# jczarnowski/DeepFactors

Measured on NVIDIA H100. Metric: keyframe-pair Jacobian+JtJ evals/sec (640x480, C=32), higher is better.
Workload: dtype f32

## Files before the change

### deepfactors_b200/csrc/dfk_api.cu

```cuda
#include <cuda_runtime.h>
#include <math.h>
#include <stdint.h>
#include <stdio.h>
#include <stdlib.h>
#include <string.h>

#include <algorithm>
#include <memory>
#include <new>
#include <string>
#include <vector>

#include "dfk.h"
#include "dfk_internal.h"

using namespace dfk;

namespace {

template <typename T, bool Pinned>
struct Scratch {
  T* ptr = nullptr;
  size_t cap = 0;

  Scratch() = default;
  Scratch(Scratch&& o) noexcept : ptr(o.ptr), cap(o.cap) { o.ptr = nullptr; o.cap = 0; }
  ~Scratch() { release(); }

  void release()
  {
    if constexpr (Pinned) cudaFreeHost(ptr);
    else cudaFree(ptr);
    ptr = nullptr;
    cap = 0;
  }
  cudaError_t ensure(size_t need)
  {
    if (cap >= need) return cudaSuccess;
    const size_t n = std::max(need, cap * 2);
    release();
    void* p = nullptr;
    const cudaError_t e = Pinned ? cudaMallocHost(&p, n * sizeof(T)) : cudaMalloc(&p, n * sizeof(T));
    if (e != cudaSuccess) return e;
    ptr = static_cast<T*>(p);
    cap = n;
    return e;
  }
};
template <typename T>
using DeviceBuf = Scratch<T, false>;
template <typename T>
using PinnedBuf = Scratch<T, true>;

}

struct DfkContext {
  int device = 0;
  int num_sms = 1;
  int sm_limit = 0;
  cudaStream_t own_stream = nullptr;
  cudaStream_t stream = nullptr;
  std::string err;
  DfkSfmAlignerParams params;
  DfkGramMode gram_mode = DFK_GRAM_AUTO;
  float se3_huber_delta = 0.1f;

  DeviceBuf<float> simple_scratch;
  DeviceBuf<unsigned int> counter;
  DeviceBuf<float> out_dev;
  PinnedBuf<float> out_host;
  DeviceBuf<float> code_dev;
  DeviceBuf<float> track_dev;
  PinnedBuf<float> track_host;
  DeviceBuf<unsigned char> batch_dev;
  PinnedBuf<unsigned char> batch_host;
  DeviceBuf<float> batch_partials;
  DeviceBuf<unsigned int> batch_counters;

  DeviceBuf<float> sparse_dev;
  PinnedBuf<float> sparse_host;
  DeviceBuf<unsigned char> rep_dev;
  std::vector<unsigned char> rep_host;
  DeviceBuf<unsigned char> geo_dev;
  std::vector<unsigned char> geo_host;
  DeviceBuf<SfmItemDev> items_dev;
  DeviceBuf<float> partials_dev;
  struct RayTab {
    float fx, fy, u0, v0;
    uint32_t w, h;
    DeviceBuf<float> dev;
    bool built;
  };
  std::vector<RayTab> ray_cache;
  std::vector<size_t> ray_pending;
  bool ray_flush = false;
  DeviceBuf<float> codes_dev;
  std::vector<float> codes_host;
  DeviceBuf<float> records_dev;
  PinnedBuf<float> records_host;
  std::vector<SfmItemDev> items_host;

  bool profiling = false;
  std::vector<cudaEvent_t> ev_pool;
  size_t ev_used = 0;
  double ev_ms_accum = 0.0;
  uint64_t ev_count_accum = 0;
  uint64_t launches = 0;

  ~DfkContext()
  {
    for (cudaEvent_t e : ev_pool) cudaEventDestroy(e);
    if (own_stream) cudaStreamDestroy(own_stream);
  }
};

struct DfkSfmStream {
  int device = 0, code_size = 0, max_items = 0, depth = 0;
  size_t max_bytes = 0;
  cudaStream_t copy_stream = nullptr;
  struct Slot {
    DeviceBuf<unsigned char> dev;
    DeviceBuf<float> rec_dev;
    PinnedBuf<float> rec_host;
    cudaEvent_t uploaded = nullptr, done = nullptr;
    int n = 0;
    uint64_t ticket = 0;
    bool busy = false;
  };
  std::vector<Slot> slots;
  std::vector<DfkSfmWorkItem> dev_items;
  uint64_t next_ticket = 0, next_wait = 0;
};

struct DfkWindow {
  int device = 0;
  WindowDev dev{};
  DeviceBuf<int> ints;
  DeviceBuf<float> areas;
  size_t floats = 0;
};

namespace {

DfkStatus fail(DfkHandle h, DfkStatus s, const std::string& msg)
{
  if (h) h->err = msg;
  return s;
}

DfkStatus oom(DfkHandle h) noexcept
{
  if (h) {
    try {
      h->err = "out of host memory";
    } catch (...) {
    }
  }
  return DFK_ERR_NOMEM;
}

template <class F>
DfkStatus guarded(DfkHandle h, F&& body) noexcept
{
  if (!h) return DFK_ERR_INVALID_ARG;
  try {
    return body();
  } catch (...) {
    return oom(h);
  }
}

DfkStatus cuda_fail(DfkHandle h, cudaError_t e, const char* what)
{
  std::string m = std::string(what) + ": " + cudaGetErrorString(e);
  cudaGetLastError();
  return fail(h, DFK_ERR_CUDA, m);
}

#define DFK_CUDA(h, call, what)                            \
  do {                                                     \
    cudaError_t e__ = (call);                              \
    if (e__ != cudaSuccess) return cuda_fail(h, e__, what); \
  } while (0)

#define DFK_TRY(call)                      \
  do {                                     \
    const DfkStatus s__ = (call);          \
    if (s__ != DFK_OK) return s__;         \
  } while (0)

DfkStatus download(DfkHandle h, void* host, const void* dev, size_t bytes, const char* copy_what, const char* sync_what)
{
  DFK_CUDA(h, cudaMemcpyAsync(host, dev, bytes, cudaMemcpyDeviceToHost, h->stream), copy_what);
  DFK_CUDA(h, cudaStreamSynchronize(h->stream), sync_what);
  return DFK_OK;
}

struct DeviceGuard {
  int prev = -1;
  explicit DeviceGuard(int dev)
  {
    cudaGetDevice(&prev);
    if (prev != dev) cudaSetDevice(dev);
    else prev = -1;
  }
  ~DeviceGuard()
  {
    if (prev >= 0) cudaSetDevice(prev);
  }
};

void quat_rotate(const float q[4], const float v[3], float out[3])
{
  float uv0 = q[1] * v[2] - q[2] * v[1];
  float uv1 = q[2] * v[0] - q[0] * v[2];
  float uv2 = q[0] * v[1] - q[1] * v[0];
  uv0 += uv0; uv1 += uv1; uv2 += uv2;
  out[0] = (v[0] + q[3] * uv0) + (q[1] * uv2 - q[2] * uv1);
  out[1] = (v[1] + q[3] * uv1) + (q[2] * uv0 - q[0] * uv2);
  out[2] = (v[2] + q[3] * uv2) + (q[0] * uv1 - q[1] * uv0);
}

void quat_mul(const float a[4], const float b[4], float o[4])
{
  const float w = a[3] * b[3] - a[0] * b[0] - a[1] * b[1] - a[2] * b[2];
  const float x = a[3] * b[0] + a[0] * b[3] + a[1] * b[2] - a[2] * b[1];
  const float y = a[3] * b[1] + a[1] * b[3] + a[2] * b[0] - a[0] * b[2];
  const float z = a[3] * b[2] + a[2] * b[3] + a[0] * b[1] - a[1] * b[0];
  o[0] = x; o[1] = y; o[2] = z; o[3] = w;
}

void quat_to_matrix(const float q[4], float R[9])
{
  const float tx = 2.f * q[0], ty = 2.f * q[1], tz = 2.f * q[2];
  const float twx = tx * q[3], twy = ty * q[3], twz = tz * q[3];
  const float txx = tx * q[0], txy = ty * q[0], txz = tz * q[0];
  const float tyy = ty * q[1], tyz = tz * q[1], tzz = tz * q[2];
  R[0] = 1.f - (tyy + tzz); R[1] = txy - twz;         R[2] = txz + twy;
  R[3] = txy + twz;         R[4] = 1.f - (txx + tzz); R[5] = tyz - twx;
  R[6] = txz - twy;         R[7] = tyz + twx;         R[8] = 1.f - (txx + tyy);
}

void relative_pose(const float a[7], const float b[7], float ab[7], float* jac_a, float* jac_b)
{
  const float qi[4] = {-a[0], -a[1], -a[2], a[3]};
  const float nta[3] = {-a[4], -a[5], -a[6]};
  float ti[3], tmp[3];
  quat_rotate(qi, nta, ti);
  quat_mul(qi, b, ab);
  quat_rotate(qi, b + 4, tmp);
  ab[4] = ti[0] + tmp[0]; ab[5] = ti[1] + tmp[1]; ab[6] = ti[2] + tmp[2];
  if (!jac_a && !jac_b) return;
  float Ra[9], RaT[9];
  quat_to_matrix(a, Ra);
  for (int i = 0; i < 3; ++i)
    for (int j = 0; j < 3; ++j) RaT[i * 3 + j] = Ra[j * 3 + i];
  if (jac_a) {
    const float d[3] = {a[4] - b[4], a[5] - b[5], a[6] - b[6]};
    float v[3];
    for (int i = 0; i < 3; ++i) v[i] = RaT[i * 3 + 0] * d[0] + RaT[i * 3 + 1] * d[1] + RaT[i * 3 + 2] * d[2];
    const float hat[9] = {0, -v[2], v[1], v[2], 0, -v[0], -v[1], v[0], 0};
    for (int i = 0; i < 36; ++i) jac_a[i] = 0.f;
    for (int i = 0; i < 3; ++i)
      for (int j = 0; j < 3; ++j) {
        float s = 0.f;
        for (int k = 0; k < 3; ++k) s += hat[i * 3 + k] * RaT[k * 3 + j];
        jac_a[i * 6 + j] = -RaT[i * 3 + j];
        jac_a[i * 6 + 3 + j] = -s;
        jac_a[(3 + i) * 6 + 3 + j] = -RaT[i * 3 + j];
      }
  }
  if (jac_b) {
    for (int i = 0; i < 36; ++i) jac_b[i] = 0.f;
    for (int i = 0; i < 3; ++i)
      for (int j = 0; j < 3; ++j) {
        jac_b[i * 6 + j] = RaT[i * 3 + j];
        jac_b[(3 + i) * 6 + 3 + j] = RaT[i * 3 + j];
      }
  }
}

bool img_ok(const DfkImage* im, uint32_t w, uint32_t h, uint32_t floats_per_px)
{
  return im && im->ptr && im->width == w && im->height == h && (im->pitch_bytes % 4 == 0) &&
         im->pitch_bytes >= (size_t)w * floats_per_px * 4;
}

bool cam_ok(const DfkCamera* cam, uint32_t w, uint32_t h)
{
  return cam && cam->width <= (float)w && cam->height <= (float)h && cam->width >= 0.0f && cam->height >= 0.0f;
}

View view_of(const DfkImage* im) { return View{static_cast<const float*>(im->ptr), (uint32_t)(im->pitch_bytes / 4)}; }

bool aligned(const void* p, size_t a) { return reinterpret_cast<uintptr_t>(p) % a == 0; }

PixelCam make_pixel_cam(const float pose[7], const DfkCamera* cam, int border, float min_dpt)
{
  PixelCam pc;
  for (int i = 0; i < 4; ++i) pc.q[i] = pose[i];
  for (int i = 0; i < 3; ++i) pc.t[i] = pose[4 + i];
  pc.fx = cam->fx; pc.fy = cam->fy; pc.u0 = cam->u0; pc.v0 = cam->v0;
  pc.border = (float)border;
  pc.ulim = cam->width - (float)border;
  pc.vlim = cam->height - (float)border;
  pc.min_dpt = min_dpt;
  return pc;
}

template <class D>
void set_relative_pose(D& d, const float pose1[7], const float pose0[7], const DfkCamera& cam)
{
  float p10[7];
  relative_pose(pose1, pose0, p10, d.P1, d.P0);
  for (int k = 0; k < 4; ++k) d.q[k] = p10[k];
  for (int k = 0; k < 3; ++k) d.t[k] = p10[4 + k];
  quat_to_matrix(p10, d.R);
  d.fx = cam.fx; d.fy = cam.fy; d.u0 = cam.u0; d.v0 = cam.v0;
}

uint32_t bits_of(float f)
{
  uint32_t u;
  memcpy(&u, &f, 4);
  return u;
}

void unpack_record(const float* rec, size_t nh, size_t np, float* JtJ, float* Jtr, float* residual, uint64_t* inliers)
{
  std::copy_n(rec, nh, JtJ);
  std::copy_n(rec + nh, np, Jtr);
  *residual = rec[nh + np];
  *inliers = bits_of(rec[nh + np + 1]);
}

bool track_level_ok(const DfkTrackLevel& L)
{
  const uint32_t W = L.img0.width, H = L.img0.height;
  return L.iterations >= 0 && W != 0 && H != 0 && img_ok(&L.img0, W, H, 1) && img_ok(&L.img1, W, H, 1) &&
         img_ok(&L.dpt0, W, H, 1) && img_ok(&L.grad1, W, H, 2) && cam_ok(&L.cam, W, H);
}

void track_outputs(const float* sys, const DfkTrackLevel& level0, float* inlier_fraction, float* error, float* last_system)
{
  if (level0.iterations > 0) {
    const uint32_t inl = bits_of(sys[28]), area = level0.img0.width * level0.img0.height;
    if (inlier_fraction) *inlier_fraction = area ? (float)inl / (float)area : 0.0f;
    if (error) *error = inl != 0 ? sys[27] / (float)inl : INFINITY;
  }
  if (last_system) memcpy(last_system, sys, sizeof(float) * 29);
}

uint32_t gcd_u32(uint32_t a, uint32_t b)
{
  while (b) {
    const uint32_t t = a % b;
    a = b;
    b = t;
  }
  return a;
}

uint32_t perm_multiplier(uint32_t n)
{
  static const bool no_perm = []() { const char* e = getenv("DFK_NO_PERM"); return e && e[0] == '1'; }();
  if (no_perm) return 1;
  if (n <= 2 || n > 65535u) return 1;
  uint32_t m = (uint32_t)((double)n * 0.6180339887498949);
  if (m < 1) m = 1;
  while (gcd_u32(m, n) != 1) ++m;
  return m % n == 0 ? 1 : m;
}

DfkStatus build_items(DfkHandle h, const DfkSfmWorkItem* items, int n, int code_size, int tile_px, int max_ctas,
                      const float* codes_dev, SfmLaunchPlan* plan)
{
  h->ray_pending.clear();
  if (h->ray_flush) {
    h->ray_cache.clear();
    h->ray_flush = false;
  }
  const DfkDenseSfmParams& sp = h->params.sfmparams;
  h->items_host.resize(n);
  uint32_t tile_cursor = 0;
  for (int i = 0; i < n; ++i) {
    const DfkSfmWorkItem& w = items[i];
    SfmItemDev& d = h->items_host[i];
    const uint32_t W = w.img0.width, H = w.img0.height;
    if (W == 0 || H == 0) return fail(h, DFK_ERR_INVALID_ARG, "[SfmAligner::RunStep] empty image");
    if (!img_ok(&w.img0, W, H, 1) || !img_ok(&w.img1, W, H, 1) || !img_ok(&w.dpt0, W, H, 1) ||
        !img_ok(&w.valid0, W, H, 1) || !img_ok(&w.prx0_jac, W, H, code_size) || !img_ok(&w.grad1, W, H, 2))
      return fail(h, DFK_ERR_INVALID_ARG,
                  "[SfmAligner::RunStep] inconsistent image views (size, pitch or null pointer) in work item " +
                      std::to_string(i));
    if (!cam_ok(&w.cam, W, H))
      return fail(h, DFK_ERR_INVALID_ARG,
                  "[SfmAligner::RunStep] camera viewport larger than the image views in work item " + std::to_string(i));
    set_relative_pose(d, w.pose1, w.pose0, w.cam);
    d.border = (float)sp.valid_border;
    d.ulim = w.cam.width - (float)sp.valid_border;
    d.vlim = w.cam.height - (float)sp.valid_border;
    d.min_dpt = sp.min_dpt; d.avg_dpt = sp.avg_dpt; d.huber_delta = sp.huber_delta;
    d.img0 = (const float*)w.img0.ptr; d.img1 = (const float*)w.img1.ptr; d.dpt0 = (const float*)w.dpt0.ptr;
    d.valid0 = (float*)w.valid0.ptr; d.jac = (const float*)w.prx0_jac.ptr; d.grad1 = (const float*)w.grad1.ptr;
    d.img0_pitch = (uint32_t)(w.img0.pitch_bytes / 4); d.img1_pitch = (uint32_t)(w.img1.pitch_bytes / 4);
    d.dpt0_pitch = (uint32_t)(w.dpt0.pitch_bytes / 4); d.valid0_pitch = (uint32_t)(w.valid0.pitch_bytes / 4);
    d.jac_pitch = (uint32_t)(w.prx0_jac.pitch_bytes / 4); d.grad1_pitch = (uint32_t)(w.grad1.pitch_bytes / 4);
    d.dpt_out = nullptr; d.dpt_out_pitch = 0; d.code = nullptr;
    const bool fused = (w.code != nullptr);
    if (fused) {
      if (!img_ok(&w.prx_orig, W, H, 1))
        return fail(h, DFK_ERR_INVALID_ARG,
                    "[SfmAligner::RunStep] fused depth decode: inconsistent prx_orig view in work item " + std::to_string(i));
      d.dpt_out = (float*)w.dpt0.ptr;
      d.dpt_out_pitch = d.dpt0_pitch;
      d.dpt0 = (const float*)w.prx_orig.ptr;
      d.dpt0_pitch = (uint32_t)(w.prx_orig.pitch_bytes / 4);
      d.code = codes_dev + (size_t)i * code_size;
      memcpy(h->codes_host.data() + (size_t)i * code_size, w.code, sizeof(float) * code_size);
    }
    d.width = W; d.height = H; d.num_pixels = W * H;
    d.num_tiles = (d.num_pixels + tile_px - 1) / tile_px;
    size_t rt = 0;
    for (const auto& r : h->ray_cache) {
      if (r.fx == d.fx && r.fy == d.fy && r.u0 == d.u0 && r.v0 == d.v0 && r.w == W && r.h == H) break;
      ++rt;
    }
    if (rt == h->ray_cache.size()) {
      if (rt >= 256) h->ray_flush = true;
      DfkContext::RayTab r{d.fx, d.fy, d.u0, d.v0, W, H, {}, false};
      if (r.dev.ensure((size_t)W + H) != cudaSuccess)
        return fail(h, DFK_ERR_CUDA, "[SfmAligner::RunStep] scratch allocation failed");
      h->ray_cache.push_back(std::move(r));
    }
    d.ray_tab = h->ray_cache[rt].dev.ptr;
    if (!h->ray_cache[rt].built) h->ray_pending.push_back(rt);
    d.tile_begin = tile_cursor;
    tile_cursor += d.num_tiles;
    d.perm_mul = perm_multiplier(d.num_tiles);
    d.mag_tiles = (uint32_t)((1ull << 32) / d.num_tiles);
    d.mag_width = (uint32_t)((1ull << 32) / W);
    d.flags = 0;
    const bool bulk = (W % 4 == 0) && aligned(d.img0, 16) && aligned(d.dpt0, 16) && aligned(d.jac, 16) &&
                      (d.img0_pitch % 4 == 0) && (d.dpt0_pitch % 4 == 0) && (d.jac_pitch % 4 == 0) &&
                      (code_size % 4 == 0);
    if (bulk) d.flags |= ITEM_FLAG_BULK;
    if (aligned(d.grad1, 8) && d.grad1_pitch % 2 == 0) d.flags |= ITEM_FLAG_GRAD_ALIGNED;
    if (fused) d.flags |= ITEM_FLAG_FUSED_DEPTH;
  }
  const int T = (int)tile_cursor;
  int G = std::min(max_ctas, T);
  if (G < 1) G = 1;
  plan->num_items = n;
  plan->num_tiles = T;
  plan->num_ctas = G;
  uint32_t partial_cursor = 0;
  int c = 0;
  for (int i = 0; i < n; ++i) {
    SfmItemDev& d = h->items_host[i];
    const long long tb = d.tile_begin, te = tb + d.num_tiles;
    while ((long long)(c + 1) * T / G <= tb) ++c;
    int first = c, last = c;
    while ((long long)(last + 1) * T / G < te) ++last;
    d.first_cta = (uint32_t)first;
    d.num_ctas = (uint32_t)(last - first + 1);
    d.partial_begin = partial_cursor;
    partial_cursor += d.num_ctas;
  }
  plan->num_partials = (int)partial_cursor;
  return DFK_OK;
}

constexpr size_t kMaxEventPairs = 8192;

DfkStatus drain_events(DfkHandle h)
{
  if (h->ev_used == 0) return DFK_OK;
  DFK_CUDA(h, cudaStreamSynchronize(h->stream), "profiling: stream synchronize failed");
  for (size_t k = 0; k < h->ev_used; ++k) {
    float ms = 0.f;
    DFK_CUDA(h, cudaEventElapsedTime(&ms, h->ev_pool[2 * k], h->ev_pool[2 * k + 1]), "profiling: event read failed");
    h->ev_ms_accum += ms;
  }
  h->ev_count_accum += h->ev_used;
  h->ev_used = 0;
  return DFK_OK;
}

DfkStatus profile_events(DfkHandle h, cudaEvent_t* e0, cudaEvent_t* e1)
{
  if (h->ev_used == kMaxEventPairs) DFK_TRY(drain_events(h));
  while (h->ev_pool.size() < 2 * (h->ev_used + 1)) {
    cudaEvent_t e;
    DFK_CUDA(h, cudaEventCreate(&e), "profiling: event creation failed");
    h->ev_pool.push_back(e);
  }
  *e0 = h->ev_pool[2 * h->ev_used];
  *e1 = h->ev_pool[2 * h->ev_used + 1];
  h->ev_used += 1;
  return DFK_OK;
}

DfkStatus run_batch(DfkHandle h, const DfkSfmWorkItem* items, int n, int code_size, float* records_dev)
{
  if (!items || n <= 0 || !records_dev) return fail(h, DFK_ERR_INVALID_ARG, "[SfmAligner::RunStep] null/empty batch");
  const bool wide = sfm_wide_supported(code_size);
  if (!sfm_fp32_supported(code_size) && !wide)
    return fail(h, DFK_ERR_UNSUPPORTED,
                "[SfmAligner::RunStep] no kernel instantiated for code size " + std::to_string(code_size));
  bool tc = (h->gram_mode == DFK_GRAM_TF32X3) || (h->gram_mode == DFK_GRAM_AUTO && sfm_tc_supported(code_size));
  if (tc) {
    bool grads_ok = true;
    for (int i = 0; i < n && grads_ok; ++i)
      grads_ok = items[i].grad1.ptr && aligned(items[i].grad1.ptr, 8) && (items[i].grad1.pitch_bytes % 8 == 0);
    if (!grads_ok) {
      if (h->gram_mode == DFK_GRAM_TF32X3)
        return fail(h, DFK_ERR_UNSUPPORTED, "[SfmAligner::RunStep] tensor-core path needs 8-byte aligned grad1 rows");
      tc = false;
    }
  }
  if (tc && !sfm_tc_supported(code_size))
    return fail(h, DFK_ERR_UNSUPPORTED,
                "[SfmAligner::RunStep] tensor-core Gram path is not instantiated for code size " +
                    std::to_string(code_size));
  DeviceGuard guard(h->device);
  SfmLaunchPlan plan;
  const int tile_px = tc ? kTcTilePixels : (wide ? sfm_wide_tile_pixels(code_size) : kTilePixels);
  bool any_fused = false;
  for (int i = 0; i < n; ++i) any_fused = any_fused || items[i].code != nullptr;
  if (any_fused) {
    DFK_CUDA(h, h->codes_dev.ensure((size_t)n * code_size), "[SfmAligner::RunStep] scratch allocation failed");
    h->codes_host.assign((size_t)n * code_size, 0.0f);
  }
  const int ctas_per_sm = tc ? kTcCtasPerSm : (wide ? 1 : sfm_fp32_ctas_per_sm(code_size));
  const int sms = (h->sm_limit > 0 && h->sm_limit < h->num_sms) ? h->sm_limit : h->num_sms;
  DFK_TRY(build_items(h, items, n, code_size, tile_px, ctas_per_sm * sms, h->codes_dev.ptr, &plan));
  if (any_fused)
    DFK_CUDA(h, cudaMemcpyAsync(h->codes_dev.ptr, h->codes_host.data(), sizeof(float) * (size_t)n * code_size,
                                cudaMemcpyHostToDevice, h->stream),
             "[SfmAligner::RunStep] code upload failed");
  const size_t pfloats = tc ? (size_t)kTcPartialFloats : sfm_partial_floats(code_size);
  DFK_CUDA(h, h->items_dev.ensure((size_t)n), "[SfmAligner::RunStep] scratch allocation failed");
  DFK_CUDA(h, h->partials_dev.ensure((size_t)plan.num_partials * pfloats), "[SfmAligner::RunStep] scratch allocation failed");
  SfmItemDev* items_dev = h->items_dev.ptr;
  float* partials_dev = h->partials_dev.ptr;
  DFK_CUDA(h, cudaMemcpyAsync(items_dev, h->items_host.data(), sizeof(SfmItemDev) * n, cudaMemcpyHostToDevice, h->stream),
           "[SfmAligner::RunStep] work list upload failed");
  if (!h->ray_pending.empty()) {
    DFK_CUDA(h, launch_sfm_ray_tables(items_dev, n, h->stream), "[SfmAligner::RunStep] kernel launch failed");
    for (size_t rt : h->ray_pending) h->ray_cache[rt].built = true;
    h->launches += 1;
  }
  cudaEvent_t ev0 = nullptr, ev1 = nullptr;
  if (h->profiling) DFK_TRY(profile_events(h, &ev0, &ev1));
  if (tc) {
    DFK_CUDA(h, launch_sfm_tc(items_dev, plan, partials_dev, h->stream, ev0, ev1),
             "[SfmAligner::RunStep] kernel launch failed");
  } else if (wide) {
    DFK_CUDA(h, launch_sfm_wide(code_size, items_dev, plan, partials_dev, h->stream, ev0, ev1),
             "[SfmAligner::RunStep] kernel launch failed");
  } else {
    DFK_CUDA(h, launch_sfm_fp32(code_size, items_dev, plan, partials_dev, h->stream, ev0, ev1),
             "[SfmAligner::RunStep] kernel launch failed");
  }
  DFK_CUDA(h, launch_sfm_finalize(code_size, tc, items_dev, n, partials_dev, records_dev, h->stream),
           "[SfmAligner::RunStep] kernel launch failed");
  h->launches += 2;
  return DFK_OK;
}

}

extern "C" {

int dfk_version(void) { return DFK_VERSION; }

const char* dfk_status_string(DfkStatus s)
{
  switch (s) {
    case DFK_OK: return "ok";
    case DFK_ERR_INVALID_ARG: return "invalid argument";
    case DFK_ERR_CUDA: return "CUDA error";
    case DFK_ERR_UNSUPPORTED: return "unsupported";
    case DFK_ERR_NOMEM: return "out of memory";
  }
  return "unknown";
}

int dfk_sfm_supports_code_size(int code_size)
{
  return (sfm_fp32_supported(code_size) || sfm_wide_supported(code_size)) ? 1 : 0;
}

DfkStatus dfk_create(int device, DfkHandle* out)
{
  try {
    if (!out) return DFK_ERR_INVALID_ARG;
    *out = nullptr;
    int count = 0;
    cudaError_t e = cudaGetDeviceCount(&count);
    if (e != cudaSuccess || count == 0) return DFK_ERR_CUDA;
    if (device < 0) {
      if (cudaGetDevice(&device) != cudaSuccess) return DFK_ERR_CUDA;
    }
    if (device >= count) return DFK_ERR_INVALID_ARG;
    DfkContext* h = new (std::nothrow) DfkContext();
    if (!h) return DFK_ERR_NOMEM;
    h->device = device;
    h->params.sfmparams = DfkDenseSfmParams{0.1f, 1000.f, 2.0f, 0.0f, 2};
    h->params.step_threads = 32; h->params.step_blocks = 11; h->params.eval_threads = 224; h->params.eval_blocks = 66;
    DeviceGuard guard(device);
    bool ok = true;
    ok = ok && cudaDeviceGetAttribute(&h->num_sms, cudaDevAttrMultiProcessorCount, device) == cudaSuccess;
    ok = ok && cudaStreamCreateWithFlags(&h->own_stream, cudaStreamNonBlocking) == cudaSuccess;
    h->stream = h->own_stream;
    ok = ok && h->simple_scratch.ensure(kSimpleScratchFloats) == cudaSuccess;
    ok = ok && h->counter.ensure(1) == cudaSuccess;
    ok = ok && h->out_dev.ensure(32) == cudaSuccess;
    ok = ok && h->code_dev.ensure(256) == cudaSuccess;
    ok = ok && h->out_host.ensure(32) == cudaSuccess;
    ok = ok && cudaMemset(h->counter.ptr, 0, sizeof(unsigned int)) == cudaSuccess;
    if (!ok) {
      dfk_destroy(h);
      return DFK_ERR_CUDA;
    }
    *out = h;
    return DFK_OK;
  } catch (...) {
    return DFK_ERR_NOMEM;
  }
}

DfkStatus dfk_destroy(DfkHandle h)
{
  if (!h) return DFK_OK;
  DeviceGuard guard(h->device);
  if (h->own_stream) cudaStreamSynchronize(h->own_stream);
  delete h;
  return DFK_OK;
}

DfkStatus dfk_set_stream(DfkHandle h, void* cuda_stream)
{
  return guarded(h, [&] {
    h->stream = static_cast<cudaStream_t>(cuda_stream);
    return DFK_OK;
  });
}

DfkStatus dfk_use_own_stream(DfkHandle h)
{
  return guarded(h, [&] {
    h->stream = h->own_stream;
    return DFK_OK;
  });
}

DfkStatus dfk_set_sm_limit(DfkHandle h, int num_sms)
{
  return guarded(h, [&] {
    if (num_sms < 0) return fail(h, DFK_ERR_INVALID_ARG, "[dfk_set_sm_limit] num_sms < 0");
    h->sm_limit = num_sms;
    return DFK_OK;
  });
}

void* dfk_get_stream(DfkHandle h) { return h ? h->stream : nullptr; }

DfkStatus dfk_synchronize(DfkHandle h)
{
  return guarded(h, [&] {
    DeviceGuard guard(h->device);
    DFK_CUDA(h, cudaStreamSynchronize(h->stream), "stream synchronize failed");
    return DFK_OK;
  });
}

const char* dfk_last_error(DfkHandle h) { return h ? h->err.c_str() : "null handle"; }

DfkStatus dfk_set_profiling(DfkHandle h, int enabled)
{
  return guarded(h, [&] {
    h->profiling = enabled != 0;
    return DFK_OK;
  });
}

DfkStatus dfk_get_profile(DfkHandle h, double* main_kernel_ms, uint64_t* main_kernel_launches,
                          uint64_t* total_kernel_launches)
{
  return guarded(h, [&] {
    DeviceGuard guard(h->device);
    DFK_TRY(drain_events(h));
    if (main_kernel_ms) *main_kernel_ms = h->ev_ms_accum;
    if (main_kernel_launches) *main_kernel_launches = h->ev_count_accum;
    if (total_kernel_launches) *total_kernel_launches = h->launches;
    h->ev_ms_accum = 0.0;
    h->ev_count_accum = 0;
    h->launches = 0;
    return DFK_OK;
  });
}

DfkStatus dfk_sfm_set_params(DfkHandle h, const DfkSfmAlignerParams* p)
{
  return guarded(h, [&] {
    if (!p) return DFK_ERR_INVALID_ARG;
    if (p->step_threads % 32 != 0 || p->eval_threads % 32 != 0)
      return fail(h, DFK_ERR_INVALID_ARG, "threads must be a multiple of 32!");
    if (p->step_blocks > 1024 || p->eval_blocks > 1024) return fail(h, DFK_ERR_INVALID_ARG, "blocks must be less than 1024");
    if (p->sfmparams.valid_border < 1)
      return fail(h, DFK_ERR_INVALID_ARG, "valid_border must be >= 1 (bilinear sampling reads ix+1, iy+1)");
    h->params = *p;
    return DFK_OK;
  });
}

DfkStatus dfk_sfm_get_params(DfkHandle h, DfkSfmAlignerParams* p)
{
  return guarded(h, [&] {
    if (!p) return DFK_ERR_INVALID_ARG;
    *p = h->params;
    return DFK_OK;
  });
}

DfkStatus dfk_sfm_set_gram_mode(DfkHandle h, DfkGramMode m)
{
  return guarded(h, [&] {
    if (m != DFK_GRAM_AUTO && m != DFK_GRAM_FP32 && m != DFK_GRAM_TF32X3)
      return fail(h, DFK_ERR_INVALID_ARG, "unknown gram mode");
    h->gram_mode = m;
    return DFK_OK;
  });
}

DfkStatus dfk_se3_set_huber_delta(DfkHandle h, float v)
{
  return guarded(h, [&] {
    h->se3_huber_delta = v;
    return DFK_OK;
  });
}

DfkStatus dfk_sfm_run_step_batch(DfkHandle h, const DfkSfmWorkItem* items, int n, int code_size, float* records_dev)
{
  return guarded(h, [&] { return run_batch(h, items, n, code_size, records_dev); });
}

DfkStatus dfk_sfm_run_step_batch_host(DfkHandle h, const DfkSfmWorkItem* items, int n, int code_size,
                                      float* records_host)
{
  return guarded(h, [&] {
    if (!records_host || n <= 0) return fail(h, DFK_ERR_INVALID_ARG, "[SfmAligner::RunStep] null/empty batch");
    if (!dfk_sfm_supports_code_size(code_size))
      return fail(h, DFK_ERR_UNSUPPORTED,
                  "[SfmAligner::RunStep] no kernel instantiated for code size " + std::to_string(code_size));
    DeviceGuard guard(h->device);
    const size_t rec = (size_t)DFK_SFM_RECORD_FLOATS(code_size);
    DFK_CUDA(h, h->records_dev.ensure(rec * n), "[SfmAligner::RunStep] scratch allocation failed");
    DFK_CUDA(h, h->records_host.ensure(rec * n), "[SfmAligner::RunStep] pinned allocation failed");
    DFK_TRY(run_batch(h, items, n, code_size, h->records_dev.ptr));
    DFK_TRY(download(h, h->records_host.ptr, h->records_dev.ptr, rec * n * sizeof(float),
                     "[SfmAligner::RunStep] result download failed", "[SfmAligner::RunStep] kernel launch failed"));
    memcpy(records_host, h->records_host.ptr, rec * n * sizeof(float));
    return DFK_OK;
  });
}

DfkStatus dfk_sfm_run_step(DfkHandle h, const float pose0[7], const float pose1[7], const float* ,
                           int code_size, const DfkCamera* cam, const DfkImage* img0, const DfkImage* img1,
                           const DfkImage* dpt0, const DfkImage* , const DfkImage* valid0,
                           const DfkImage* prx0_jac, const DfkImage* grad1, float* JtJ, float* Jtr, float* residual,
                           uint64_t* inliers)
{
  return guarded(h, [&] {
    if (!pose0 || !pose1 || !cam || !img0 || !img1 || !dpt0 || !valid0 || !prx0_jac || !grad1 || !JtJ || !Jtr ||
        !residual || !inliers)
      return fail(h, DFK_ERR_INVALID_ARG, "[SfmAligner::RunStep] null argument");
    DfkSfmWorkItem w{};
    memcpy(w.pose0, pose0, sizeof(w.pose0));
    memcpy(w.pose1, pose1, sizeof(w.pose1));
    w.cam = *cam;
    w.img0 = *img0; w.img1 = *img1; w.dpt0 = *dpt0; w.valid0 = *valid0; w.prx0_jac = *prx0_jac; w.grad1 = *grad1;
    const int NP = 12 + code_size;
    const int NH = NP * (NP + 1) / 2;
    std::vector<float> rec((size_t)DFK_SFM_RECORD_FLOATS(code_size));
    DFK_TRY(dfk_sfm_run_step_batch_host(h, &w, 1, code_size, rec.data()));
    unpack_record(rec.data(), NH, NP, JtJ, Jtr, residual, inliers);
    return DFK_OK;
  });
}

static DfkStatus fetch_out(DfkHandle h, int nfloats, const char* what)
{
  h->launches += 1;
  return download(h, h->out_host.ptr, h->out_dev.ptr, sizeof(float) * nfloats, what, what);
}

DfkStatus dfk_sfm_evaluate_error(DfkHandle h, const float pose0[7], const float pose1[7], const DfkCamera* cam,
                                 const DfkImage* img0, const DfkImage* img1, const DfkImage* dpt0,
                                 const DfkImage* , const DfkImage* , float* residual,
                                 uint64_t* inliers)
{
  return guarded(h, [&] {
    if (!pose0 || !pose1 || !cam || !img0 || !img1 || !dpt0 || !residual || !inliers)
      return fail(h, DFK_ERR_INVALID_ARG, "[SfmAligner::EvaluateError] null argument");
    const uint32_t W = img0->width, H = img0->height;
    if (W == 0 || H == 0 || !img_ok(img0, W, H, 1) || !img_ok(img1, W, H, 1) || !img_ok(dpt0, W, H, 1))
      return fail(h, DFK_ERR_INVALID_ARG, "[SfmAligner::EvaluateError] inconsistent image views");
    if (!cam_ok(cam, W, H)) return fail(h, DFK_ERR_INVALID_ARG, "[SfmAligner::EvaluateError] camera viewport larger than the image views");
    DeviceGuard guard(h->device);
    float p10[7];
    relative_pose(pose1, pose0, p10, nullptr, nullptr);
    const PixelCam pc = make_pixel_cam(p10, cam, 1, 0.0f);
    DFK_CUDA(h, launch_eval_error(pc, h->params.sfmparams.huber_delta, (int)W, (int)H, view_of(img0), view_of(img1),
                                  view_of(dpt0), h->simple_scratch.ptr, h->counter.ptr, h->out_dev.ptr, h->stream),
             "[SfmAligner::EvaluateError] kernel launch failed");
    DFK_TRY(fetch_out(h, 2, "[SfmAligner::EvaluateError] kernel launch failed"));
    unpack_record(h->out_host.ptr, 0, 0, nullptr, nullptr, residual, inliers);
    return DFK_OK;
  });
}

DfkStatus dfk_se3_run_step(DfkHandle h, const float se3[7], const DfkCamera* cam, const DfkImage* img0,
                           const DfkImage* img1, const DfkImage* dpt0, const DfkImage* grad1, float* JtJ, float* Jtr,
                           float* residual, uint64_t* inliers)
{
  return guarded(h, [&] {
    if (!se3 || !cam || !img0 || !img1 || !dpt0 || !grad1 || !JtJ || !Jtr || !residual || !inliers)
      return fail(h, DFK_ERR_INVALID_ARG, "[SE3Aligner::RunStep] null argument");
    const uint32_t W = img0->width, H = img0->height;
    if (W == 0 || H == 0 || !img_ok(img0, W, H, 1) || !img_ok(img1, W, H, 1) || !img_ok(dpt0, W, H, 1) ||
        !img_ok(grad1, W, H, 2))
      return fail(h, DFK_ERR_INVALID_ARG, "[SE3Aligner::RunStep] inconsistent image views");
    if (!cam_ok(cam, W, H)) return fail(h, DFK_ERR_INVALID_ARG, "[SE3Aligner::RunStep] camera viewport larger than the image views");
    DeviceGuard guard(h->device);
    const PixelCam pc = make_pixel_cam(se3, cam, 1, 0.0f);
    const View g = view_of(grad1);
    const bool galigned = aligned(g.ptr, 8) && g.pitch % 2 == 0;
    DFK_CUDA(h, launch_se3_step(pc, h->se3_huber_delta, (int)W, (int)H, view_of(img0), view_of(img1), view_of(dpt0), g,
                                galigned, h->simple_scratch.ptr, h->counter.ptr, h->out_dev.ptr, h->stream),
             "[SE3Aligner::RunStep] Kernel launch failed");
    DFK_TRY(fetch_out(h, 29, "[SE3Aligner::RunStep] Kernel launch failed"));
    unpack_record(h->out_host.ptr, 21, 6, JtJ, Jtr, residual, inliers);
    return DFK_OK;
  });
}

DfkStatus dfk_se3_track(DfkHandle h, float pose_ck[7], const DfkTrackLevel* levels, int num_levels,
                        float* inlier_fraction, float* error, float* last_system, float* history, int history_capacity)
{
  return guarded(h, [&] {
    if (!pose_ck || !levels || num_levels <= 0)
      return fail(h, DFK_ERR_INVALID_ARG, "[CameraTracker::TrackFrame] null argument / no pyramid levels");
    int total_iters = 0;
    for (int l = 0; l < num_levels; ++l) {
      if (!track_level_ok(levels[l]))
        return fail(h, DFK_ERR_INVALID_ARG,
                    "[CameraTracker::TrackFrame] inconsistent image views / camera larger than them / negative iteration count at level " +
                        std::to_string(l));
      total_iters += levels[l].iterations;
    }
    if (history && history_capacity < total_iters)
      return fail(h, DFK_ERR_INVALID_ARG, "[CameraTracker::TrackFrame] history buffer too small");
    DeviceGuard guard(h->device);
    const size_t nfloat = 8 + 36 * (size_t)std::max(total_iters, 1);
    DFK_CUDA(h, h->track_dev.ensure(nfloat), "[CameraTracker::TrackFrame] scratch allocation failed");
    DFK_CUDA(h, h->track_host.ensure(nfloat + 32), "[CameraTracker::TrackFrame] pinned allocation failed");
    float* track_dev = h->track_dev.ptr;
    float* track_host = h->track_host.ptr;
    memcpy(track_host, pose_ck, sizeof(float) * 7);
    DFK_CUDA(h, cudaMemcpyAsync(track_dev, track_host, sizeof(float) * 7, cudaMemcpyHostToDevice, h->stream),
             "[CameraTracker::TrackFrame] pose upload failed");
    DFK_CUDA(h, cudaMemsetAsync(h->out_dev.ptr, 0, sizeof(float) * 32, h->stream), "[CameraTracker::TrackFrame] memset failed");
    int it = 0;
    for (int l = num_levels - 1; l >= 0; --l) {
      const DfkTrackLevel& L = levels[l];
      const PixelCam pc = make_pixel_cam(pose_ck, &L.cam, 1, 0.0f);
      const View g = view_of(&L.grad1);
      const bool galigned = aligned(g.ptr, 8) && g.pitch % 2 == 0;
      for (int k = 0; k < L.iterations; ++k, ++it) {
        DFK_CUDA(h, launch_se3_step(pc, h->se3_huber_delta, (int)L.img0.width, (int)L.img0.height, view_of(&L.img0),
                                    view_of(&L.img1), view_of(&L.dpt0), g, galigned, h->simple_scratch.ptr,
                                    h->counter.ptr, h->out_dev.ptr, h->stream, track_dev, track_dev + 8 + 36 * (size_t)it),
                 "[CameraTracker::TrackFrame] kernel launch failed");
        h->launches += 1;
      }
    }
    float* host_sys = track_host + nfloat;
    DFK_CUDA(h, cudaMemcpyAsync(track_host, track_dev, sizeof(float) * (8 + 36 * (size_t)total_iters),
                                cudaMemcpyDeviceToHost, h->stream),
             "[CameraTracker::TrackFrame] read-back failed");
    DFK_TRY(download(h, host_sys, h->out_dev.ptr, sizeof(float) * 29, "[CameraTracker::TrackFrame] read-back failed",
                     "[CameraTracker::TrackFrame] stream synchronize failed"));
    memcpy(pose_ck, track_host, sizeof(float) * 7);
    track_outputs(host_sys, levels[0], inlier_fraction, error, last_system);
    if (history) memcpy(history, track_host + 8, sizeof(float) * 36 * (size_t)total_iters);
    return DFK_OK;
  });
}

DfkStatus dfk_se3_track_batch(DfkHandle h, int num_problems, int num_levels, float* poses_ck,
                              const DfkTrackLevel* levels, float* inlier_fraction, float* error, float* last_systems)
{
  return guarded(h, [&] {
    if (!poses_ck || !levels || num_levels <= 0)
      return fail(h, DFK_ERR_INVALID_ARG, "[CameraTracker::TrackFrame batch] null argument / no pyramid levels");
    if (num_problems < 1 || num_problems > 65535)
      return fail(h, DFK_ERR_INVALID_ARG, "[CameraTracker::TrackFrame batch] number of problems must be in [1, 65535]");
    const int N = num_problems, L = num_levels;
    std::vector<Se3TrackDesc> descs((size_t)L * N);
    std::vector<int> level_blocks(L, 0);
    int stride = 1;
    for (int n = 0; n < N; ++n) {
      for (int l = 0; l < L; ++l) {
        const DfkTrackLevel& T = levels[(size_t)n * L + l];
        if (!track_level_ok(T))
          return fail(h, DFK_ERR_INVALID_ARG,
                      "[CameraTracker::TrackFrame batch] inconsistent image views / camera larger than them / "
                      "negative iteration count at problem " + std::to_string(n) + " level " + std::to_string(l));
        if (T.iterations != levels[l].iterations)
          return fail(h, DFK_ERR_INVALID_ARG,
                      "[CameraTracker::TrackFrame batch] problem " + std::to_string(n) + " has " +
                          std::to_string(T.iterations) + " iterations at level " + std::to_string(l) +
                          ", problem 0 has " + std::to_string(levels[l].iterations));
        Se3TrackDesc& d = descs[(size_t)l * N + n];
        d.pc = make_pixel_cam(poses_ck + 7 * (size_t)n, &T.cam, 1, 0.0f);
        d.img0 = view_of(&T.img0); d.img1 = view_of(&T.img1); d.dpt0 = view_of(&T.dpt0); d.grad1 = view_of(&T.grad1);
        d.width = (int)T.img0.width;
        d.height = (int)T.img0.height;
        d.nblocks = se3_step_blocks(d.width, d.height);
        d.grad_aligned = aligned(d.grad1.ptr, 8) && d.grad1.pitch % 2 == 0;
        level_blocks[l] = std::max(level_blocks[l], d.nblocks);
        stride = std::max(stride, d.nblocks);
      }
    }
    DeviceGuard guard(h->device);
    const size_t desc_bytes = (descs.size() * sizeof(Se3TrackDesc) + 15) & ~(size_t)15;
    const size_t pose_bytes = sizeof(float) * 8 * (size_t)N, out_bytes = sizeof(float) * 32 * (size_t)N;
// ... 689 lines not shown
```

### deepfactors_b200/csrc/dfk_window.cu

```cuda
#include <cuda_runtime.h>
#include <stdint.h>

#include "dfk_internal.h"

namespace dfk {

namespace {

__device__ __forceinline__ int packed_index(int i, int j, int NP) { return i * NP - (i * (i - 1)) / 2 + (j - i); }
__device__ __forceinline__ float rec_h(const float* rec, int a, int b, int NP)
{
  return a <= b ? rec[packed_index(a, b, NP)] : rec[packed_index(b, a, NP)];
}

__device__ __forceinline__ int link_row0(int r) { return r < 6 ? r : 6 + r; }
__device__ __forceinline__ int link_row1(int r, int C) { return r < 6 ? 6 + r : 6 + C + r; }

__global__ void __launch_bounds__(256)
window_assemble_kernel(WindowDev w, const float* __restrict__ records, const float* __restrict__ geo,
                       float* __restrict__ out)
{
  const int C = w.code_size, B = 6 + C, NP = 12 + C;
  const int NH = NP * (NP + 1) / 2, REC = NH + NP + 2;
  const int NG = 12 + 2 * C, NHG = NG * (NG + 1) / 2, RECG = NHG + NG + 2;
  float* tail = out + (size_t)w.num_keyframes * (B * B + B) + (size_t)w.num_pairs * B * 6;
  const int job = blockIdx.x;
  if (job < w.num_keyframes) {
    const int k = job;
    float* D = out + (size_t)k * B * B;
    float* g = out + (size_t)w.num_keyframes * B * B + (size_t)k * B;
    const int a0 = w.kf0_ptr[k], a1 = w.kf0_ptr[k + 1];
    const int b0 = w.kf1_ptr[k], b1 = w.kf1_ptr[k + 1];
    const int l00 = w.lk0_ptr[k], l01 = w.lk0_ptr[k + 1];
    const int l10 = w.lk1_ptr[k], l11 = w.lk1_ptr[k + 1];
    for (int e = threadIdx.x; e < B * B + B; e += blockDim.x) {
      float s = 0.0f;
      if (e < B * B) {
        const int r = e / B, c = e - r * B;
        const int lr = r < 6 ? r : 6 + r, lc = c < 6 ? c : 6 + c;
        for (int q = a0; q < a1; ++q) s += rec_h(records + (size_t)w.kf0_items[q] * REC, lr, lc, NP);
        if (r < 6 && c < 6)
          for (int q = b0; q < b1; ++q) s += rec_h(records + (size_t)w.kf1_items[q] * REC, 6 + r, 6 + c, NP);
        for (int q = l00; q < l01; ++q) s += rec_h(geo + (size_t)w.lk0_links[q] * RECG, link_row0(r), link_row0(c), NG);
        for (int q = l10; q < l11; ++q)
          s += rec_h(geo + (size_t)w.lk1_links[q] * RECG, link_row1(r, C), link_row1(c, C), NG);
        D[e] = s;
      } else {
        const int r = e - B * B;
        const int lr = r < 6 ? r : 6 + r;
        for (int q = a0; q < a1; ++q) s -= records[(size_t)w.kf0_items[q] * REC + NH + lr];
        if (r < 6)
          for (int q = b0; q < b1; ++q) s -= records[(size_t)w.kf1_items[q] * REC + NH + 6 + r];
        for (int q = l00; q < l01; ++q) s -= geo[(size_t)w.lk0_links[q] * RECG + NHG + link_row0(r)];
        for (int q = l10; q < l11; ++q) s -= geo[(size_t)w.lk1_links[q] * RECG + NHG + link_row1(r, C)];
        g[r] = s;
      }
    }
  } else if (job < w.num_keyframes + w.num_pairs) {
    const int p = job - w.num_keyframes;
    float* O = out + (size_t)w.num_keyframes * (B * B + B) + (size_t)p * B * 6;
    const int i0 = w.pair_ptr[p], i1 = w.pair_ptr[p + 1];
    for (int e = threadIdx.x; e < B * 6; e += blockDim.x) {
      const int r = e / 6, c = e - r * 6;
      const int lr = r < 6 ? r : 6 + r;
      float s = 0.0f;
      for (int q = i0; q < i1; ++q) s += rec_h(records + (size_t)w.pair_items[q] * REC, lr, 6 + c, NP);
      O[e] = s;
    }
  } else if (job < w.num_keyframes + w.num_pairs + w.num_links) {
    const int l = job - w.num_keyframes - w.num_pairs;
    float* O = tail + 2 + (size_t)l * B * B;
    const float* rec = geo + (size_t)l * RECG;
    for (int e = threadIdx.x; e < B * B; e += blockDim.x) {
      const int r = e / B, c = e - r * B;
      O[e] = rec_h(rec, link_row0(r), link_row1(c, C), NG);
    }
  } else {
    __shared__ float red_f[8], red_i[8];
    float f = 0.0f, ni = 0.0f;
    for (int i = threadIdx.x; i < w.num_items; i += blockDim.x) {
      const float* rec = records + (size_t)i * REC;
      const uint32_t inl = __float_as_uint(rec[NH + NP + 1]);
      if (w.item_area[i] == 0.0f) {
        f += rec[NH + NP];
      } else {
        if (inl > 0) f += rec[NH + NP] / (float)inl * w.item_area[i];
        ni += (float)inl;
      }
    }
    for (int l = threadIdx.x; l < w.num_links; l += blockDim.x) f += geo[(size_t)l * RECG + NHG + NG];
    for (int o = 16; o > 0; o >>= 1) {
      f += __shfl_xor_sync(0xffffffffu, f, o);
      ni += __shfl_xor_sync(0xffffffffu, ni, o);
    }
    if ((threadIdx.x & 31) == 0) {
      red_f[threadIdx.x >> 5] = f;
      red_i[threadIdx.x >> 5] = ni;
    }
    __syncthreads();
    if (threadIdx.x == 0) {
      float sf = 0.0f, si = 0.0f;
      for (int k = 0; k < (int)(blockDim.x >> 5); ++k) {
        sf += red_f[k];
        si += red_i[k];
      }
      tail[0] = sf;
      tail[1] = si;
    }
  }
}

}

cudaError_t launch_window_assemble(const WindowDev& w, const float* records_dev, const float* geo_records_dev,
                                   float* out_dev, cudaStream_t stream)
{
  window_assemble_kernel<<<w.num_keyframes + w.num_pairs + w.num_links + 1, 256, 0, stream>>>(w, records_dev,
                                                                                             geo_records_dev, out_dev);
  return cudaGetLastError();
}

}
```

Before: 31170.

## Double-buffer work-list uploads on a side stream and split window assembly

Result: faster. 31960 (median of 6 runs) (+2.5%).

```diff
diff --git a/deepfactors_b200/csrc/dfk_api.cu b/deepfactors_b200/csrc/dfk_api.cu
--- a/deepfactors_b200/csrc/dfk_api.cu
+++ b/deepfactors_b200/csrc/dfk_api.cu
@@ -83,7 +83,6 @@
   std::vector<unsigned char> rep_host;
   DeviceBuf<unsigned char> geo_dev;
   std::vector<unsigned char> geo_host;
-  DeviceBuf<SfmItemDev> items_dev;
   DeviceBuf<float> partials_dev;
   struct RayTab {
     float fx, fy, u0, v0;
@@ -94,11 +93,20 @@
   std::vector<RayTab> ray_cache;
   std::vector<size_t> ray_pending;
   bool ray_flush = false;
-  DeviceBuf<float> codes_dev;
-  std::vector<float> codes_host;
   DeviceBuf<float> records_dev;
   PinnedBuf<float> records_host;
-  std::vector<SfmItemDev> items_host;
+  static constexpr int kItemSlots = 4;
+  struct ItemSlot {
+    PinnedBuf<SfmItemDev> host;
+    DeviceBuf<SfmItemDev> dev;
+    PinnedBuf<float> codes_host;
+    DeviceBuf<float> codes_dev;
+    cudaEvent_t uploaded = nullptr;
+    cudaEvent_t consumed = nullptr;
+  };
+  ItemSlot item_slots[kItemSlots];
+  uint64_t item_batches = 0;
+  cudaStream_t upload_stream = nullptr;
 
   bool profiling = false;
   std::vector<cudaEvent_t> ev_pool;
@@ -110,6 +118,11 @@
   ~DfkContext()
   {
     for (cudaEvent_t e : ev_pool) cudaEventDestroy(e);
+    for (ItemSlot& sl : item_slots) {
+      if (sl.uploaded) cudaEventDestroy(sl.uploaded);
+      if (sl.consumed) cudaEventDestroy(sl.consumed);
+    }
+    if (upload_stream) cudaStreamDestroy(upload_stream);
     if (own_stream) cudaStreamDestroy(own_stream);
   }
 };
@@ -373,7 +386,7 @@
 }
 
 DfkStatus build_items(DfkHandle h, const DfkSfmWorkItem* items, int n, int code_size, int tile_px, int max_ctas,
-                      const float* codes_dev, SfmLaunchPlan* plan)
+                      SfmItemDev* items_out, float* codes_out, const float* codes_dev, SfmLaunchPlan* plan)
 {
   h->ray_pending.clear();
   if (h->ray_flush) {
@@ -381,11 +394,10 @@
     h->ray_flush = false;
   }
   const DfkDenseSfmParams& sp = h->params.sfmparams;
-  h->items_host.resize(n);
   uint32_t tile_cursor = 0;
   for (int i = 0; i < n; ++i) {
     const DfkSfmWorkItem& w = items[i];
-    SfmItemDev& d = h->items_host[i];
+    SfmItemDev& d = items_out[i];
     const uint32_t W = w.img0.width, H = w.img0.height;
     if (W == 0 || H == 0) return fail(h, DFK_ERR_INVALID_ARG, "[SfmAligner::RunStep] empty image");
     if (!img_ok(&w.img0, W, H, 1) || !img_ok(&w.img1, W, H, 1) || !img_ok(&w.dpt0, W, H, 1) ||
@@ -417,7 +429,7 @@
       d.dpt0 = (const float*)w.prx_orig.ptr;
       d.dpt0_pitch = (uint32_t)(w.prx_orig.pitch_bytes / 4);
       d.code = codes_dev + (size_t)i * code_size;
-      memcpy(h->codes_host.data() + (size_t)i * code_size, w.code, sizeof(float) * code_size);
+      memcpy(codes_out + (size_t)i * code_size, w.code, sizeof(float) * code_size);
     }
     d.width = W; d.height = H; d.num_pixels = W * H;
     d.num_tiles = (d.num_pixels + tile_px - 1) / tile_px;
@@ -457,7 +469,7 @@
   uint32_t partial_cursor = 0;
   int c = 0;
   for (int i = 0; i < n; ++i) {
-    SfmItemDev& d = h->items_host[i];
+    SfmItemDev& d = items_out[i];
     const long long tb = d.tile_begin, te = tb + d.num_tiles;
     while ((long long)(c + 1) * T / G <= tb) ++c;
     int first = c, last = c;
@@ -528,24 +540,34 @@
   const int tile_px = tc ? kTcTilePixels : (wide ? sfm_wide_tile_pixels(code_size) : kTilePixels);
   bool any_fused = false;
   for (int i = 0; i < n; ++i) any_fused = any_fused || items[i].code != nullptr;
+  DfkContext::ItemSlot& sl = h->item_slots[h->item_batches % DfkContext::kItemSlots];
+  DFK_CUDA(h, cudaEventSynchronize(sl.uploaded), "[SfmAligner::RunStep] work list slot wait failed");
+  DFK_CUDA(h, sl.host.ensure((size_t)n), "[SfmAligner::RunStep] pinned allocation failed");
+  DFK_CUDA(h, sl.dev.ensure((size_t)n), "[SfmAligner::RunStep] scratch allocation failed");
+  const size_t code_floats = any_fused ? (size_t)n * code_size : 0;
   if (any_fused) {
-    DFK_CUDA(h, h->codes_dev.ensure((size_t)n * code_size), "[SfmAligner::RunStep] scratch allocation failed");
-    h->codes_host.assign((size_t)n * code_size, 0.0f);
+    DFK_CUDA(h, sl.codes_host.ensure(code_floats), "[SfmAligner::RunStep] pinned allocation failed");
+    DFK_CUDA(h, sl.codes_dev.ensure(code_floats), "[SfmAligner::RunStep] scratch allocation failed");
+    memset(sl.codes_host.ptr, 0, sizeof(float) * code_floats);
   }
   const int ctas_per_sm = tc ? kTcCtasPerSm : (wide ? 1 : sfm_fp32_ctas_per_sm(code_size));
   const int sms = (h->sm_limit > 0 && h->sm_limit < h->num_sms) ? h->sm_limit : h->num_sms;
-  DFK_TRY(build_items(h, items, n, code_size, tile_px, ctas_per_sm * sms, h->codes_dev.ptr, &plan));
+  DFK_TRY(build_items(h, items, n, code_size, tile_px, ctas_per_sm * sms, sl.host.ptr, sl.codes_host.ptr,
+                      sl.codes_dev.ptr, &plan));
+  const size_t pfloats = tc ? (size_t)kTcPartialFloats : sfm_partial_floats(code_size);
+  DFK_CUDA(h, h->partials_dev.ensure((size_t)plan.num_partials * pfloats), "[SfmAligner::RunStep] scratch allocation failed");
+  SfmItemDev* items_dev = sl.dev.ptr;
+  float* partials_dev = h->partials_dev.ptr;
+  DFK_CUDA(h, cudaStreamWaitEvent(h->upload_stream, sl.consumed, 0), "[SfmAligner::RunStep] stream wait failed");
+  DFK_CUDA(h, cudaMemcpyAsync(items_dev, sl.host.ptr, sizeof(SfmItemDev) * n, cudaMemcpyHostToDevice, h->upload_stream),
+           "[SfmAligner::RunStep] work list upload failed");
   if (any_fused)
-    DFK_CUDA(h, cudaMemcpyAsync(h->codes_dev.ptr, h->codes_host.data(), sizeof(float) * (size_t)n * code_size,
-                                cudaMemcpyHostToDevice, h->stream),
+    DFK_CUDA(h, cudaMemcpyAsync(sl.codes_dev.ptr, sl.codes_host.ptr, sizeof(float) * code_floats, cudaMemcpyHostToDevice,
+                                h->upload_stream),
              "[SfmAligner::RunStep] code upload failed");
-  const size_t pfloats = tc ? (size_t)kTcPartialFloats : sfm_partial_floats(code_size);
-  DFK_CUDA(h, h->items_dev.ensure((size_t)n), "[SfmAligner::RunStep] scratch allocation failed");
-  DFK_CUDA(h, h->partials_dev.ensure((size_t)plan.num_partials * pfloats), "[SfmAligner::RunStep] scratch allocation failed");
-  SfmItemDev* items_dev = h->items_dev.ptr;
-  float* partials_dev = h->partials_dev.ptr;
-  DFK_CUDA(h, cudaMemcpyAsync(items_dev, h->items_host.data(), sizeof(SfmItemDev) * n, cudaMemcpyHostToDevice, h->stream),
-           "[SfmAligner::RunStep] work list upload failed");
+  DFK_CUDA(h, cudaEventRecord(sl.uploaded, h->upload_stream), "[SfmAligner::RunStep] event record failed");
+  DFK_CUDA(h, cudaStreamWaitEvent(h->stream, sl.uploaded, 0), "[SfmAligner::RunStep] stream wait failed");
+  h->item_batches += 1;
   if (!h->ray_pending.empty()) {
     DFK_CUDA(h, launch_sfm_ray_tables(items_dev, n, h->stream), "[SfmAligner::RunStep] kernel launch failed");
     for (size_t rt : h->ray_pending) h->ray_cache[rt].built = true;
@@ -565,6 +587,7 @@
   }
   DFK_CUDA(h, launch_sfm_finalize(code_size, tc, items_dev, n, partials_dev, records_dev, h->stream),
            "[SfmAligner::RunStep] kernel launch failed");
+  DFK_CUDA(h, cudaEventRecord(sl.consumed, h->stream), "[SfmAligner::RunStep] event record failed");
   h->launches += 2;
   return DFK_OK;
 }
@@ -614,6 +637,11 @@
     ok = ok && cudaDeviceGetAttribute(&h->num_sms, cudaDevAttrMultiProcessorCount, device) == cudaSuccess;
     ok = ok && cudaStreamCreateWithFlags(&h->own_stream, cudaStreamNonBlocking) == cudaSuccess;
     h->stream = h->own_stream;
+    ok = ok && cudaStreamCreateWithFlags(&h->upload_stream, cudaStreamNonBlocking) == cudaSuccess;
+    for (DfkContext::ItemSlot& sl : h->item_slots) {
+      ok = ok && cudaEventCreateWithFlags(&sl.uploaded, cudaEventDisableTiming) == cudaSuccess;
+      ok = ok && cudaEventCreateWithFlags(&sl.consumed, cudaEventDisableTiming) == cudaSuccess;
+    }
     ok = ok && h->simple_scratch.ensure(kSimpleScratchFloats) == cudaSuccess;
     ok = ok && h->counter.ensure(1) == cudaSuccess;
     ok = ok && h->out_dev.ensure(32) == cudaSuccess;
@@ -636,6 +664,9 @@
   if (!h) return DFK_OK;
   DeviceGuard guard(h->device);
   if (h->own_stream) cudaStreamSynchronize(h->own_stream);
+  if (h->upload_stream) cudaStreamSynchronize(h->upload_stream);
+  for (const DfkContext::ItemSlot& sl : h->item_slots)
+    if (sl.consumed) cudaEventSynchronize(sl.consumed);
   delete h;
   return DFK_OK;
 }
diff --git a/deepfactors_b200/csrc/dfk_window.cu b/deepfactors_b200/csrc/dfk_window.cu
--- a/deepfactors_b200/csrc/dfk_window.cu
+++ b/deepfactors_b200/csrc/dfk_window.cu
@@ -16,59 +16,80 @@
 __device__ __forceinline__ int link_row0(int r) { return r < 6 ? r : 6 + r; }
 __device__ __forceinline__ int link_row1(int r, int C) { return r < 6 ? 6 + r : 6 + C + r; }
 
-__global__ void __launch_bounds__(256)
+constexpr int kAssembleThreads = 256;
+constexpr int kGatherBatch = 8;
+
+__device__ __forceinline__ int rec_h_off(int a, int b, int NP) { return a <= b ? packed_index(a, b, NP) : packed_index(b, a, NP); }
+
+template <bool Sub>
+__device__ __forceinline__ float gather_sum(float s, const float* __restrict__ recs, int stride, int off,
+                                            const int* __restrict__ list, int q0, int q1)
+{
+  for (int q = q0; q < q1; q += kGatherBatch) {
+    float v[kGatherBatch];
+#pragma unroll
+    for (int u = 0; u < kGatherBatch; ++u) v[u] = q + u < q1 ? recs[(size_t)list[q + u] * stride + off] : 0.0f;
+#pragma unroll
+    for (int u = 0; u < kGatherBatch; ++u)
+      if (q + u < q1) s = Sub ? s - v[u] : s + v[u];
+  }
+  return s;
+}
+
+__host__ __device__ __forceinline__ int keyframe_splits(int B) { return (B * B + B + kAssembleThreads - 1) / kAssembleThreads; }
+
+__global__ void __launch_bounds__(kAssembleThreads)
 window_assemble_kernel(WindowDev w, const float* __restrict__ records, const float* __restrict__ geo,
                        float* __restrict__ out)
 {
+  cudaGridDependencySynchronize();
   const int C = w.code_size, B = 6 + C, NP = 12 + C;
   const int NH = NP * (NP + 1) / 2, REC = NH + NP + 2;
   const int NG = 12 + 2 * C, NHG = NG * (NG + 1) / 2, RECG = NHG + NG + 2;
   float* tail = out + (size_t)w.num_keyframes * (B * B + B) + (size_t)w.num_pairs * B * 6;
-  const int job = blockIdx.x;
-  if (job < w.num_keyframes) {
-    const int k = job;
+  const int S = keyframe_splits(B);
+  const int job = blockIdx.x - w.num_keyframes * S;
+  if (job < 0) {
+    const int k = blockIdx.x / S;
     float* D = out + (size_t)k * B * B;
     float* g = out + (size_t)w.num_keyframes * B * B + (size_t)k * B;
     const int a0 = w.kf0_ptr[k], a1 = w.kf0_ptr[k + 1];
     const int b0 = w.kf1_ptr[k], b1 = w.kf1_ptr[k + 1];
     const int l00 = w.lk0_ptr[k], l01 = w.lk0_ptr[k + 1];
     const int l10 = w.lk1_ptr[k], l11 = w.lk1_ptr[k + 1];
-    for (int e = threadIdx.x; e < B * B + B; e += blockDim.x) {
+    for (int e = (blockIdx.x % S) * blockDim.x + threadIdx.x; e < B * B + B; e += S * blockDim.x) {
       float s = 0.0f;
       if (e < B * B) {
         const int r = e / B, c = e - r * B;
         const int lr = r < 6 ? r : 6 + r, lc = c < 6 ? c : 6 + c;
-        for (int q = a0; q < a1; ++q) s += rec_h(records + (size_t)w.kf0_items[q] * REC, lr, lc, NP);
-        if (r < 6 && c < 6)
-          for (int q = b0; q < b1; ++q) s += rec_h(records + (size_t)w.kf1_items[q] * REC, 6 + r, 6 + c, NP);
-        for (int q = l00; q < l01; ++q) s += rec_h(geo + (size_t)w.lk0_links[q] * RECG, link_row0(r), link_row0(c), NG);
-        for (int q = l10; q < l11; ++q)
-          s += rec_h(geo + (size_t)w.lk1_links[q] * RECG, link_row1(r, C), link_row1(c, C), NG);
+        s = gather_sum<false>(s, records, REC, rec_h_off(lr, lc, NP), w.kf0_items, a0, a1);
+        if (r < 6 && c < 6) s = gather_sum<false>(s, records, REC, rec_h_off(6 + r, 6 + c, NP), w.kf1_items, b0, b1);
+        if (l01 > l00)
+          s = gather_sum<false>(s, geo, RECG, rec_h_off(link_row0(r), link_row0(c), NG), w.lk0_links, l00, l01);
+        if (l11 > l10)
+          s = gather_sum<false>(s, geo, RECG, rec_h_off(link_row1(r, C), link_row1(c, C), NG), w.lk1_links, l10, l11);
         D[e] = s;
       } else {
         const int r = e - B * B;
         const int lr = r < 6 ? r : 6 + r;
-        for (int q = a0; q < a1; ++q) s -= records[(size_t)w.kf0_items[q] * REC + NH + lr];
-        if (r < 6)
-          for (int q = b0; q < b1; ++q) s -= records[(size_t)w.kf1_items[q] * REC + NH + 6 + r];
-        for (int q = l00; q < l01; ++q) s -= geo[(size_t)w.lk0_links[q] * RECG + NHG + link_row0(r)];
-        for (int q = l10; q < l11; ++q) s -= geo[(size_t)w.lk1_links[q] * RECG + NHG + link_row1(r, C)];
+        s = gather_sum<true>(s, records, REC, NH + lr, w.kf0_items, a0, a1);
+        if (r < 6) s = gather_sum<true>(s, records, REC, NH + 6 + r, w.kf1_items, b0, b1);
+        if (l01 > l00) s = gather_sum<true>(s, geo, RECG, NHG + link_row0(r), w.lk0_links, l00, l01);
+        if (l11 > l10) s = gather_sum<true>(s, geo, RECG, NHG + link_row1(r, C), w.lk1_links, l10, l11);
         g[r] = s;
       }
     }
-  } else if (job < w.num_keyframes + w.num_pairs) {
-    const int p = job - w.num_keyframes;
+  } else if (job < w.num_pairs) {
+    const int p = job;
     float* O = out + (size_t)w.num_keyframes * (B * B + B) + (size_t)p * B * 6;
     const int i0 = w.pair_ptr[p], i1 = w.pair_ptr[p + 1];
     for (int e = threadIdx.x; e < B * 6; e += blockDim.x) {
       const int r = e / 6, c = e - r * 6;
       const int lr = r < 6 ? r : 6 + r;
-      float s = 0.0f;
-      for (int q = i0; q < i1; ++q) s += rec_h(records + (size_t)w.pair_items[q] * REC, lr, 6 + c, NP);
-      O[e] = s;
+      O[e] = gather_sum<false>(0.0f, records, REC, rec_h_off(lr, 6 + c, NP), w.pair_items, i0, i1);
     }
-  } else if (job < w.num_keyframes + w.num_pairs + w.num_links) {
-    const int l = job - w.num_keyframes - w.num_pairs;
+  } else if (job < w.num_pairs + w.num_links) {
+    const int l = job - w.num_pairs;
     float* O = tail + 2 + (size_t)l * B * B;
     const float* rec = geo + (size_t)l * RECG;
     for (int e = threadIdx.x; e < B * B; e += blockDim.x) {
@@ -115,9 +136,17 @@
 cudaError_t launch_window_assemble(const WindowDev& w, const float* records_dev, const float* geo_records_dev,
                                    float* out_dev, cudaStream_t stream)
 {
-  window_assemble_kernel<<<w.num_keyframes + w.num_pairs + w.num_links + 1, 256, 0, stream>>>(w, records_dev,
-                                                                                             geo_records_dev, out_dev);
-  return cudaGetLastError();
+  cudaLaunchConfig_t cfg{};
+  cfg.gridDim = dim3(w.num_keyframes * keyframe_splits(6 + w.code_size) + w.num_pairs + w.num_links + 1);
+  cfg.blockDim = dim3(kAssembleThreads);
+  cfg.dynamicSmemBytes = 0;
+  cfg.stream = stream;
+  cudaLaunchAttribute attr[1];
+  attr[0].id = cudaLaunchAttributeProgrammaticStreamSerialization;
+  attr[0].val.programmaticStreamSerializationAllowed = 1;
+  cfg.attrs = attr;
+  cfg.numAttrs = 1;
+  return cudaLaunchKernelEx(&cfg, window_assemble_kernel, w, records_dev, geo_records_dev, out_dev);
 }
 
 }
```
